# Shuijing725/CrowdNav_Prediction_AttnGraph

Measured on AMD Instinct MI355X. Metric: env-steps/sec (sim+policy fwd) at 20 humans, higher is better.
Workload: dtype f32 (big GEMMs as bf16x3 split-precision MFMA, fp32 accumulate); 1 GPU; BASELINE configs[1]: CrowdSimVarNum-v0, 20 humans, 4096 parallel envs per GPU, HH+HR attention on, policy forward + ORCA sim step + auto-reset per step; envs_per_gpu=4096, humans=20, parallelism=dp1 (envs sharded, no rollout collective), policy_init=orthogonal, torch.manual_seed(425), sampled_actions=True, side_stream_tail=inline, dephase_steps=240

## Files before the change

crowdnav_prediction_attngraph_amd/csrc/rn_fused.hip:

```cpp
#include "rn_fused.h"
#include "row_plan.h"

namespace {

typedef float f32x4 __attribute__((ext_vector_type(4)));
typedef __bf16 bf16x8 __attribute__((ext_vector_type(8)));

constexpr int TE = 16;
constexpr int S512 = 516, S384 = 388, S128 = 132;
constexpr int O_R0 = 0;
constexpr int O_R1 = O_R0 + TE * S512;
constexpr int O_R2 = O_R1 + TE * S512;
constexpr int O_R3 = O_R2 + TE * S384;
constexpr int O_R4 = O_R3 + TE * S384;
constexpr int O_R5 = O_R4 + TE * S128;
constexpr int LDS_FLOATS = O_R5 + TE * S128;

__device__ __forceinline__ f32x4 mfma32(bf16x8 a, bf16x8 b, f32x4 c) { return __builtin_amdgcn_mfma_f32_16x16x32_bf16(a, b, c, 0, 0, 0); }

enum { A_NONE = 0, A_RELU = 1, A_TANH = 2 };

__device__ __forceinline__ float fast_tanh(float x)
{
    const float e = __builtin_amdgcn_exp2f(x * 2.88539008177792681472f);
    return 1.0f - 2.0f / (1.0f + e);
}
__device__ __forceinline__ float fast_sigmoid(float x) { return 1.0f / (1.0f + __builtin_amdgcn_exp2f(x * -1.44269504088896340736f)); }

template <int K, int NFB, int ACT>
__device__ __forceinline__ void stage(const float *__restrict__ Wfrag_, int fb_first, int fb_step, const float *__restrict__ bias, const float *in, int in_stride,
                                      float *out, int out_stride, int out_off, int relu_from, int lane)
{
    const bf16x8 *__restrict__ Wfrag = reinterpret_cast<const bf16x8 *>(Wfrag_);
    const int i = lane & 15, g = lane >> 4;
    constexpr int KS = K / 32;
    bf16x8 bh, bl;
    auto split = [&](int ks, bf16x8 &h, bf16x8 &l) {
        const f32x4 x0 = *reinterpret_cast<const f32x4 *>(in + i * in_stride + 32 * ks + 8 * g);
        const f32x4 x1 = *reinterpret_cast<const f32x4 *>(in + i * in_stride + 32 * ks + 8 * g + 4);
#pragma unroll
        for (int u = 0; u < 4; ++u) {
            const __bf16 h0 = (__bf16)x0[u], h1 = (__bf16)x1[u];
            h[u] = h0; h[4 + u] = h1;
            l[u] = (__bf16)(x0[u] - (float)h0); l[4 + u] = (__bf16)(x1[u] - (float)h1);
        }
    };
    f32x4 acc[NFB];
#pragma unroll
    for (int j = 0; j < NFB; ++j) acc[j] = f32x4{0.f, 0.f, 0.f, 0.f};
    constexpr int PF = KS < 2 ? KS : 2;
    bf16x8 ah[PF][NFB], al[PF][NFB];
#pragma unroll
    for (int p = 0; p < PF - 1; ++p)
#pragma unroll
        for (int j = 0; j < NFB; ++j) {
            const size_t base = ((size_t)(fb_first + j * fb_step) * KS + (p < KS ? p : KS - 1)) * 128 + lane;
            ah[p][j] = Wfrag[base]; al[p][j] = Wfrag[base + 64];
        }
#pragma unroll
    for (int ks = 0; ks < KS; ++ks) {
        const int kp = ks + PF - 1 < KS ? ks + PF - 1 : KS - 1;
#pragma unroll
        for (int j = 0; j < NFB; ++j) {
            const size_t base = ((size_t)(fb_first + j * fb_step) * KS + kp) * 128 + lane;
            ah[(ks + PF - 1) % PF][j] = Wfrag[base]; al[(ks + PF - 1) % PF][j] = Wfrag[base + 64];
        }
        split(ks, bh, bl);
        __builtin_amdgcn_sched_barrier(0);
#pragma unroll
        for (int j = 0; j < NFB; ++j) {
            acc[j] = mfma32(al[ks % PF][j], bh, acc[j]);
            acc[j] = mfma32(ah[ks % PF][j], bl, acc[j]);
            acc[j] = mfma32(ah[ks % PF][j], bh, acc[j]);
        }
        __builtin_amdgcn_sched_barrier(0);
    }
#pragma unroll
    for (int j = 0; j < NFB; ++j) {
        const int f0 = (fb_first + j * fb_step) * 16 + 4 * g;
        f32x4 v = acc[j];
        if (bias) v += *reinterpret_cast<const f32x4 *>(bias + f0);
#pragma unroll
        for (int q = 0; q < 4; ++q) {
            if (ACT == A_RELU) { if (f0 + q >= relu_from) v[q] = fmaxf(v[q], 0.0f); }
            if (ACT == A_TANH) v[q] = fast_tanh(v[q]);
        }
        *reinterpret_cast<f32x4 *>(out + i * out_stride + out_off + f0) = v;
    }
}

__global__ __launch_bounds__(512, 4) void rn_fused_kernel(int E, int H, RnFusedArgs a)
{
    const CnStampScope stamp_scope(a.stamp);
    extern __shared__ __attribute__((aligned(16))) float smem[];
    __builtin_amdgcn_s_setprio(3);
    const int tid = threadIdx.x, lane = tid & 63, wave = __builtin_amdgcn_readfirstlane(tid >> 6);
    const int e0 = blockIdx.x * TE;
    float *R0 = smem + O_R0, *R1 = smem + O_R1, *R2 = smem + O_R2, *R3 = smem + O_R3, *R4 = smem + O_R4, *R5 = smem + O_R5;
    const int w4 = wave & 3, hi = wave >> 2;
    int r0q[2], r1q[2];
#pragma unroll
    for (int q = 0; q < 2; ++q) {
        const int e = e0 + 2 * wave + q < E ? e0 + 2 * wave + q : E - 1;
        r0q[q] = a.row_off[e]; r1q[q] = a.row_off[e + 1];
    }
    {
        const int n = tid & 255;
        float w[9];
#pragma unroll
        for (int d = 0; d < 9; ++d) w[d] = a.rl_w[n * 9 + d];
        const float bn = a.rl_b[n];
        for (int i = (tid >> 8) * (TE / 2); i < (tid >> 8) * (TE / 2) + TE / 2; ++i) {
            const int e = e0 + i < E ? e0 + i : E - 1;
            float acc = bn;
            acc += a.temporal[e * 2] * w[0];
            acc += a.temporal[e * 2 + 1] * w[1];
#pragma unroll
            for (int d = 0; d < 7; ++d) acc += a.robot_node[e * 7 + d] * w[2 + d];
            acc = fmaxf(acc, 0.0f);
            R0[i * S512 + n] = acc;
            if (a.tap_robot && e0 + i < E) a.tap_robot[(size_t)(e0 + i) * 256 + n] = acc;
        }
        for (int idx = tid; idx < TE * 128; idx += 512) {
            const int i = idx >> 7, c = idx & 127;
            const int e = e0 + i < E ? e0 + i : E - 1;
            R4[i * S128 + c] = a.hxs_in[(size_t)e * 128 + c];
        }
    }
#pragma unroll
    for (int q = 0; q < 2; ++q) { r0q[q] = held_uniform(r0q[q]); r1q[q] = held_uniform(r1q[q]); }
    __syncthreads();
    if (hi == 0) {
        stage<256, 3, A_RELU>(a.f_te, w4, 4, a.te_b, R0, S512, R1, S512, 0, 256, lane);
        stage<256, 2, A_RELU>(a.f_te, w4 + 12, 4, a.te_b, R0, S512, R1, S512, 0, 256, lane);
    } else {
        stage<128, 3, A_NONE>(a.f_whh, w4, 4, nullptr, R4, S128, R2, S384, 0, 0, lane);
        stage<128, 3, A_NONE>(a.f_whh, w4 + 12, 4, nullptr, R4, S128, R2, S384, 0, 0, lane);
    }
    __syncthreads();
    {
        constexpr int CH = 8;
        int ndq[2];
        float x[2][CH][4];
#pragma unroll
        for (int q = 0; q < 2; ++q) ndq[q] = r1q[q] - r0q[q];
#pragma unroll
        for (int q = 0; q < 2; ++q)
#pragma unroll
            for (int u = 0; u < CH; ++u) {
                const float *row = a.out_sp + (size_t)(r0q[q] + (u < ndq[q] ? u : ndq[q] - 1)) * 256;
                x[q][u][0] = row[lane]; x[q][u][1] = row[64 + lane]; x[q][u][2] = row[128 + lane]; x[q][u][3] = row[192 + lane];
            }
#pragma unroll
        for (int q = 0; q < 2; ++q) {
            const int i = 2 * wave + q;
            const int r0 = r0q[q], nd = ndq[q];
            const float *ue = R1 + i * S512;
            const float u0 = ue[lane], u1 = ue[64 + lane], u2 = ue[128 + lane], u3 = ue[192 + lane];
            float s = -INFINITY;
#pragma unroll
            for (int u = 0; u < CH; ++u) {
                const float tot = wv_sum(u0 * x[q][u][0] + u1 * x[q][u][1] + u2 * x[q][u][2] + u3 * x[q][u][3]);
                if (lane == u && u < nd) s = tot * ((float)H / 8.0f);
            }
            for (int j0 = CH; j0 < nd; j0 += CH) {
                float y[CH][4];
#pragma unroll
                for (int u = 0; u < CH; ++u) {
                    const float *row = a.out_sp + (size_t)(r0 + (j0 + u < nd ? j0 + u : nd - 1)) * 256;
                    y[u][0] = row[lane]; y[u][1] = row[64 + lane]; y[u][2] = row[128 + lane]; y[u][3] = row[192 + lane];
                }
#pragma unroll
                for (int u = 0; u < CH; ++u) {
                    const float tot = wv_sum(u0 * y[u][0] + u1 * y[u][1] + u2 * y[u][2] + u3 * y[u][3]);
                    if (lane == j0 + u && j0 + u < nd) s = tot * ((float)H / 8.0f);
                }
            }
            const float mx = wv_max(s);
            const float p = lane < nd ? expf(s - mx) : 0.0f;
            const float denom = wv_sum(p);
            const float at = p / denom;
            if (a.tap_attn && lane < H && e0 + i < E) a.tap_attn[(size_t)(e0 + i) * H + lane] = at;
            float o0 = 0.f, o1 = 0.f, o2 = 0.f, o3 = 0.f;
#pragma unroll
            for (int u = 0; u < CH; ++u) {
                const float aj = u < nd ? wv_readlane(at, u) : 0.0f;
                if (u < nd) { o0 += aj * x[q][u][0]; o1 += aj * x[q][u][1]; o2 += aj * x[q][u][2]; o3 += aj * x[q][u][3]; }
            }
            for (int j0 = CH; j0 < nd; j0 += CH) {
                float y[CH][4];
#pragma unroll
                for (int u = 0; u < CH; ++u) {
                    const float *row = a.out_sp + (size_t)(r0 + (j0 + u < nd ? j0 + u : nd - 1)) * 256;
                    y[u][0] = row[lane]; y[u][1] = row[64 + lane]; y[u][2] = row[128 + lane]; y[u][3] = row[192 + lane];
                }
#pragma unroll
                for (int u = 0; u < CH; ++u) {
                    const float aj = wv_readlane(at, j0 + u < nd ? j0 + u : 0);
                    if (j0 + u < nd) { o0 += aj * y[u][0]; o1 += aj * y[u][1]; o2 += aj * y[u][2]; o3 += aj * y[u][3]; }
                }
            }
            float *o = R0 + i * S512;
            o[lane] = o0; o[64 + lane] = o1; o[128 + lane] = o2; o[192 + lane] = o3;
            if (a.tap_hr && e0 + i < E) {
                float *t = a.tap_hr + (size_t)(e0 + i) * 256;
                t[lane] = o0; t[64 + lane] = o1; t[128 + lane] = o2; t[192 + lane] = o3;
            }
        }
    }
    __syncthreads();
    if (hi == 0) stage<256, 1, A_RELU>(a.f_edge, w4, 4, a.edge_b, R0, S512, R1, S512, 320, 0, lane);
    __syncthreads();
    stage<128, 3, A_NONE>(a.f_wih, wave, 8, a.bih, R1 + 256, S512, R3, S384, 0, 0, lane);
    __syncthreads();
    for (int idx = tid; idx < TE * 128; idx += 512) {
        const int i = idx >> 7, c = idx & 127;
        const int e = e0 + i < E ? e0 + i : E - 1;
        const float m = a.masks[e];
        const float *gie = R3 + i * S384, *ghe = R2 + i * S384;
        const float hr = m * ghe[c] + a.bhh[c], hz = m * ghe[128 + c] + a.bhh[128 + c], hn = m * ghe[256 + c] + a.bhh[256 + c];
        const float r = fast_sigmoid(gie[c] + hr);
        const float z = fast_sigmoid(gie[128 + c] + hz);
        const float n = fast_tanh(gie[256 + c] + r * hn);
        const float h = m * R4[i * S128 + c];
        const float hnew = (1.0f - z) * n + z * h;
        R5[i * S128 + c] = hnew;
        if (e0 + i < E) a.hxs_out[(size_t)(e0 + i) * 128 + c] = hnew;
    }
    __syncthreads();
    stage<128, 4, A_TANH>(a.f_ac0, wave, 8, a.ac0_b, R5, S128, R0, S512, 0, 0, lane);
    __syncthreads();
    {
        const float *fw = hi == 0 ? a.f_a2 : a.f_c2, *fb = hi == 0 ? a.a2_b : a.c2_b;
        const float *src = hi == 0 ? R0 : R0 + 256;
        stage<256, 2, A_TANH>(fw, w4, 4, fb, src, S512, R1, S512, hi * 256, 0, lane);
        stage<256, 2, A_TANH>(fw, w4 + 8, 4, fb, src, S512, R1, S512, hi * 256, 0, lane);
    }
    __syncthreads();
    for (int q = 0; q < 2; ++q) {
        const int i = 2 * wave + q;
        if (e0 + i >= E) break;
        const int e = e0 + i;
        const float *av = R1 + i * S512, *cv = av + 256;
        float sv = 0.f, s0 = 0.f, s1 = 0.f;
#pragma unroll
        for (int k = 0; k < 4; ++k) {
            const int d = lane + 64 * k;
            sv += cv[d] * a.cl_w[d];
            s0 += av[d] * a.fm_w[d];
            s1 += av[d] * a.fm_w[256 + d];
            if (a.tap_actor) a.tap_actor[(size_t)e * 256 + d] = av[d];
        }
        sv = wv_sum(sv); s0 = wv_sum(s0); s1 = wv_sum(s1);
        if (lane == 0) {
            a.value[e] = sv + a.cl_b[0];
            if (a.action) {
                const float mean0 = s0 + a.fm_b[0], mean1 = s1 + a.fm_b[1];
                const float ls0 = a.logstd[0], ls1 = a.logstd[1];
                const float sd0 = expf(ls0), sd1 = expf(ls1);
                const float a0 = a.eps ? mean0 + sd0 * a.eps[2 * e] : mean0;
                const float a1 = a.eps ? mean1 + sd1 * a.eps[2 * e + 1] : mean1;
                a.action[2 * e] = a0; a.action[2 * e + 1] = a1;
                const float HALF_LOG_2PI = 0.91893853320467274178f;
                const float d0 = a0 - mean0, d1 = a1 - mean1;
                a.logp[e] = (-(d0 * d0) / (2.0f * sd0 * sd0) - ls0 - HALF_LOG_2PI) + (-(d1 * d1) / (2.0f * sd1 * sd1) - ls1 - HALF_LOG_2PI);
            }
        }
    }
}

__global__ void rn_bake_kernel(int N, int K, const float *__restrict__ w, __bf16 *__restrict__ out)
{
    const size_t idx = (size_t)blockIdx.x * blockDim.x + threadIdx.x;
    if (idx >= (size_t)N * K) return;
    const int u = idx & 7, lane = (idx >> 3) & 63;
    const size_t rest = idx >> 9;
    const int KS = K / 32;
    const int ks = (int)(rest % KS), fb = (int)(rest / KS);
    const float x = w[(size_t)(fb * 16 + (lane & 15)) * K + 32 * ks + 8 * (lane >> 4) + u];
    const __bf16 hi = (__bf16)x;
    const size_t base = (((size_t)fb * KS + ks) * 2) * 512 + lane * 8 + u;
    out[base] = hi;
    out[base + 512] = (__bf16)(x - (float)hi);
}

}

int rn_fused_bake(int N, int K, const float *w, float *out, hipStream_t st)
{
    CN_REQUIRE(N % 16 == 0 && K % 32 == 0, "rn_fused_bake: N must be a multiple of 16, K of 32");
    const size_t n = (size_t)N * K;
    hipLaunchKernelGGL(rn_bake_kernel, dim3((unsigned)((n + 255) / 256)), dim3(256), 0, st, N, K, w, reinterpret_cast<__bf16 *>(out));
    CN_CHECK_LAUNCH();
    return CN_OK;
}

int rn_fused_forward(int E, int H, const RnFusedArgs &args, hipStream_t st)
{
    constexpr size_t lds = (size_t)LDS_FLOATS * sizeof(float);
    static thread_local int attr_dev = -1;
    int dev = 0;
    CN_HIP(hipGetDevice(&dev));
    if (dev != attr_dev) {
        CN_HIP(hipFuncSetAttribute(reinterpret_cast<const void *>(&rn_fused_kernel), hipFuncAttributeMaxDynamicSharedMemorySize, (int)lds));
        attr_dev = dev;
    }
    RnFusedArgs a = args;
    a.stamp = cn_stamp_slot(CN_K_RN_FUSED);
    hipLaunchKernelGGL(rn_fused_kernel, dim3((E + TE - 1) / TE), dim3(512), lds, st, E, H, a);
    CN_CHECK_LAUNCH();
    return CN_OK;
}
```

Before: 15.65 million env-steps/s.

## Preload biases, head weights and per-env scalars into LDS; rebalance GEMM waves

All biases, head weights, masks, eps and small scalars are loaded once at kernel start into a new LDS region, with loads issued up front and held in registers, replacing scattered global reads later in the kernel. Robot-node inputs are loaded per wave and broadcast with readlane. The first stage now splits work 5/3 across waves between the te and whh GEMMs, and the a2/c2 stage uses one call with four fragment blocks. Tap writes are compiled out through a template flag. The cost is more LDS per block and more register pressure up front.

```diff
diff --git a/crowdnav_prediction_attngraph_amd/csrc/rn_fused.hip b/crowdnav_prediction_attngraph_amd/csrc/rn_fused.hip
--- a/crowdnav_prediction_attngraph_amd/csrc/rn_fused.hip
+++ b/crowdnav_prediction_attngraph_amd/csrc/rn_fused.hip
@@ -14,7 +14,15 @@
 constexpr int O_R3 = O_R2 + TE * S384;
 constexpr int O_R4 = O_R3 + TE * S384;
 constexpr int O_R5 = O_R4 + TE * S128;
-constexpr int LDS_FLOATS = O_R5 + TE * S128;
+constexpr int O_T = O_R5 + TE * S128;
+constexpr int T_TEB = 0, T_EDGEB = T_TEB + 320, T_BIH = T_EDGEB + 64, T_BHH = T_BIH + 384, T_AC0B = T_BHH + 384, T_A2B = T_AC0B + 512;
+constexpr int T_C2B = T_A2B + 256, T_CLW = T_C2B + 256, T_FMW = T_CLW + 256;
+constexpr int T_VEC4 = (T_FMW + 512) / 4;
+constexpr int T_SM = T_FMW + 512;
+constexpr int SM_MASK = 0, SM_EPS = 16, SM_CLB = 48, SM_FMB = 49, SM_LS = 51, SM_WORDS = 53;
+constexpr int T_FLOATS = T_SM + 64;
+constexpr int LDS_FLOATS = O_T + T_FLOATS;
+static_assert(LDS_FLOATS * sizeof(float) <= 160 * 1024, "rn_fused: LDS");
 
 __device__ __forceinline__ f32x4 mfma32(bf16x8 a, bf16x8 b, f32x4 c) { return __builtin_amdgcn_mfma_f32_16x16x32_bf16(a, b, c, 0, 0, 0); }
 
@@ -27,8 +35,8 @@
 }
 __device__ __forceinline__ float fast_sigmoid(float x) { return 1.0f / (1.0f + __builtin_amdgcn_exp2f(x * -1.44269504088896340736f)); }
 
-template <int K, int NFB, int ACT>
-__device__ __forceinline__ void stage(const float *__restrict__ Wfrag_, int fb_first, int fb_step, const float *__restrict__ bias, const float *in, int in_stride,
+template <int K, int NFB, int ACT, bool BIAS>
+__device__ __forceinline__ void stage(const float *__restrict__ Wfrag_, int fb_first, int fb_step, const float *bias, const float *in, int in_stride,
                                       float *out, int out_stride, int out_off, int relu_from, int lane)
 {
     const bf16x8 *__restrict__ Wfrag = reinterpret_cast<const bf16x8 *>(Wfrag_);
@@ -79,7 +87,7 @@
     for (int j = 0; j < NFB; ++j) {
         const int f0 = (fb_first + j * fb_step) * 16 + 4 * g;
         f32x4 v = acc[j];
-        if (bias) v += *reinterpret_cast<const f32x4 *>(bias + f0);
+        if (BIAS) v += *reinterpret_cast<const f32x4 *>(bias + f0);
 #pragma unroll
         for (int q = 0; q < 4; ++q) {
             if (ACT == A_RELU) { if (f0 + q >= relu_from) v[q] = fmaxf(v[q], 0.0f); }
@@ -89,6 +97,7 @@
     }
 }
 
+template <bool TAPS>
 __global__ __launch_bounds__(512, 4) void rn_fused_kernel(int E, int H, RnFusedArgs a)
 {
     const CnStampScope stamp_scope(a.stamp);
@@ -96,7 +105,7 @@
     __builtin_amdgcn_s_setprio(3);
     const int tid = threadIdx.x, lane = tid & 63, wave = __builtin_amdgcn_readfirstlane(tid >> 6);
     const int e0 = blockIdx.x * TE;
-    float *R0 = smem + O_R0, *R1 = smem + O_R1, *R2 = smem + O_R2, *R3 = smem + O_R3, *R4 = smem + O_R4, *R5 = smem + O_R5;
+    float *R0 = smem + O_R0, *R1 = smem + O_R1, *R2 = smem + O_R2, *R3 = smem + O_R3, *R4 = smem + O_R4, *R5 = smem + O_R5, *T = smem + O_T;
     const int w4 = wave & 3, hi = wave >> 2;
     int r0q[2], r1q[2];
 #pragma unroll
@@ -104,38 +113,97 @@
         const int e = e0 + 2 * wave + q < E ? e0 + 2 * wave + q : E - 1;
         r0q[q] = a.row_off[e]; r1q[q] = a.row_off[e + 1];
     }
-    {
-        const int n = tid & 255;
-        float w[9];
-#pragma unroll
-        for (int d = 0; d < 9; ++d) w[d] = a.rl_w[n * 9 + d];
-        const float bn = a.rl_b[n];
-        for (int i = (tid >> 8) * (TE / 2); i < (tid >> 8) * (TE / 2) + TE / 2; ++i) {
-            const int e = e0 + i < E ? e0 + i : E - 1;
+    const int n = tid & 255;
+    float w[9];
+#pragma unroll
+    for (int d = 0; d < 9; ++d) w[d] = a.rl_w[n * 9 + d];
+    float bn = a.rl_b[n];
+    float obs_t, obs_r;
+    {
+        const int lt = lane < 16 ? lane : 15, lr = lane < 56 ? lane : 55;
+        const int it = e0 + 8 * hi + (lt >> 1), ir = e0 + 8 * hi + lr / 7;
+        obs_t = a.temporal[(size_t)(it < E ? it : E - 1) * 2 + (lt & 1)];
+        obs_r = a.robot_node[(size_t)(ir < E ? ir : E - 1) * 7 + lr % 7];
+    }
+    float hx[4];
+#pragma unroll
+    for (int k = 0; k < 4; ++k) {
+        const int i = (tid >> 7) + 4 * k;
+        hx[k] = a.hxs_in[(size_t)(e0 + i < E ? e0 + i : E - 1) * 128 + (tid & 127)];
+    }
+    f32x4 tv[2];
+    {
+        const float *const p_teb = a.te_b, *const p_edgeb = a.edge_b, *const p_bih = a.bih, *const p_bhh = a.bhh, *const p_ac0b = a.ac0_b;
+        const float *const p_a2b = a.a2_b, *const p_c2b = a.c2_b, *const p_clw = a.cl_w, *const p_fmw = a.fm_w;
+#pragma unroll
+        for (int r = 0; r < 2; ++r) {
+            const int j = 512 * r + tid < T_VEC4 ? 512 * r + tid : T_VEC4 - 1, f = 4 * j;
+            const float *src = p_teb; int first = T_TEB;
+            src = f >= T_EDGEB ? p_edgeb : src; first = f >= T_EDGEB ? T_EDGEB : first;
+            src = f >= T_BIH ? p_bih : src; first = f >= T_BIH ? T_BIH : first;
+            src = f >= T_BHH ? p_bhh : src; first = f >= T_BHH ? T_BHH : first;
+            src = f >= T_AC0B ? p_ac0b : src; first = f >= T_AC0B ? T_AC0B : first;
+            src = f >= T_A2B ? p_a2b : src; first = f >= T_A2B ? T_A2B : first;
+            src = f >= T_C2B ? p_c2b : src; first = f >= T_C2B ? T_C2B : first;
+            src = f >= T_CLW ? p_clw : src; first = f >= T_CLW ? T_CLW : first;
+            src = f >= T_FMW ? p_fmw : src; first = f >= T_FMW ? T_FMW : first;
+            tv[r] = *reinterpret_cast<const f32x4 *>(src + (f - first));
+        }
+    }
+    float smw;
+    {
+        const float *const p_masks = a.masks, *const p_eps = a.eps, *const p_clb = a.cl_b, *const p_fmb = a.fm_b, *const p_ls = a.logstd;
+        const bool has_eps = p_eps != nullptr;
+        const int sl = lane < SM_WORDS ? lane : SM_WORDS - 1;
+        const int i = sl < SM_EPS ? sl : (sl - SM_EPS) >> 1;
+        const int e = e0 + i < E ? e0 + i : E - 1;
+        const bool is_eps = sl >= SM_EPS && has_eps;
+        const float *src = is_eps ? p_eps : p_masks; int off = is_eps ? 2 * e + (sl & 1) : e;
+        src = sl >= SM_CLB ? p_clb : src; off = sl >= SM_CLB ? 0 : off;
+        src = sl >= SM_FMB ? p_fmb : src; off = sl >= SM_FMB ? sl - SM_FMB : off;
+        src = sl >= SM_LS ? p_ls : src; off = sl >= SM_LS ? sl - SM_LS : off;
+        smw = src[off];
+    }
+#pragma unroll
+    for (int d = 0; d < 9; ++d) w[d] = held(w[d]);
+    bn = held(bn); obs_t = held(obs_t); obs_r = held(obs_r); smw = held(smw);
+#pragma unroll
+    for (int k = 0; k < 4; ++k) hx[k] = held(hx[k]);
+#pragma unroll
+    for (int r = 0; r < 2; ++r) tv[r] = held(tv[r]);
+#pragma unroll
+    for (int q = 0; q < 2; ++q) { r0q[q] = held_uniform(r0q[q]); r1q[q] = held_uniform(r1q[q]); }
+    *reinterpret_cast<f32x4 *>(T + 4 * tid) = tv[0];
+    if (512 + tid < T_VEC4) *reinterpret_cast<f32x4 *>(T + 4 * (512 + tid)) = tv[1];
+    if (wave == 0) T[T_SM + lane] = smw;
+#pragma unroll
+    for (int k = 0; k < 4; ++k) R4[((tid >> 7) + 4 * k) * S128 + (tid & 127)] = hx[k];
+    {
+        float rs[TE / 2];
+#pragma unroll
+        for (int ii = 0; ii < TE / 2; ++ii) {
             float acc = bn;
-            acc += a.temporal[e * 2] * w[0];
-            acc += a.temporal[e * 2 + 1] * w[1];
-#pragma unroll
-            for (int d = 0; d < 7; ++d) acc += a.robot_node[e * 7 + d] * w[2 + d];
-            acc = fmaxf(acc, 0.0f);
-            R0[i * S512 + n] = acc;
-            if (a.tap_robot && e0 + i < E) a.tap_robot[(size_t)(e0 + i) * 256 + n] = acc;
-        }
-        for (int idx = tid; idx < TE * 128; idx += 512) {
-            const int i = idx >> 7, c = idx & 127;
-            const int e = e0 + i < E ? e0 + i : E - 1;
-            R4[i * S128 + c] = a.hxs_in[(size_t)e * 128 + c];
-        }
-    }
-#pragma unroll
-    for (int q = 0; q < 2; ++q) { r0q[q] = held_uniform(r0q[q]); r1q[q] = held_uniform(r1q[q]); }
-    __syncthreads();
-    if (hi == 0) {
-        stage<256, 3, A_RELU>(a.f_te, w4, 4, a.te_b, R0, S512, R1, S512, 0, 256, lane);
-        stage<256, 2, A_RELU>(a.f_te, w4 + 12, 4, a.te_b, R0, S512, R1, S512, 0, 256, lane);
+            acc += wv_readlane(obs_t, 2 * ii) * w[0];
+            acc += wv_readlane(obs_t, 2 * ii + 1) * w[1];
+#pragma unroll
+            for (int d = 0; d < 7; ++d) acc += wv_readlane(obs_r, 7 * ii + d) * w[2 + d];
+            rs[ii] = fmaxf(acc, 0.0f);
+            R0[(8 * hi + ii) * S512 + n] = rs[ii];
+        }
+        if (TAPS) {
+#pragma unroll
+            for (int ii = 0; ii < TE / 2; ++ii) {
+                const int i = 8 * hi + ii;
+                if (e0 + i < E) a.tap_robot[(size_t)(e0 + i) * 256 + n] = rs[ii];
+            }
+        }
+    }
+    __syncthreads();
+    if (wave < 5) {
+        stage<256, 4, A_RELU, true>(a.f_te, wave, 5, T + T_TEB, R0, S512, R1, S512, 0, 256, lane);
     } else {
-        stage<128, 3, A_NONE>(a.f_whh, w4, 4, nullptr, R4, S128, R2, S384, 0, 0, lane);
-        stage<128, 3, A_NONE>(a.f_whh, w4 + 12, 4, nullptr, R4, S128, R2, S384, 0, 0, lane);
+        stage<128, 4, A_NONE, false>(a.f_whh, wave - 5, 3, nullptr, R4, S128, R2, S384, 0, 0, lane);
+        stage<128, 4, A_NONE, false>(a.f_whh, wave - 5 + 12, 3, nullptr, R4, S128, R2, S384, 0, 0, lane);
     }
     __syncthreads();
     {
@@ -180,7 +248,6 @@
             const float p = lane < nd ? expf(s - mx) : 0.0f;
             const float denom = wv_sum(p);
             const float at = p / denom;
-            if (a.tap_attn && lane < H && e0 + i < E) a.tap_attn[(size_t)(e0 + i) * H + lane] = at;
             float o0 = 0.f, o1 = 0.f, o2 = 0.f, o3 = 0.f;
 #pragma unroll
             for (int u = 0; u < CH; ++u) {
@@ -202,69 +269,72 @@
             }
             float *o = R0 + i * S512;
             o[lane] = o0; o[64 + lane] = o1; o[128 + lane] = o2; o[192 + lane] = o3;
-            if (a.tap_hr && e0 + i < E) {
+            if (TAPS && e0 + i < E) {
+                if (lane < H) a.tap_attn[(size_t)(e0 + i) * H + lane] = at;
                 float *t = a.tap_hr + (size_t)(e0 + i) * 256;
                 t[lane] = o0; t[64 + lane] = o1; t[128 + lane] = o2; t[192 + lane] = o3;
             }
         }
     }
     __syncthreads();
-    if (hi == 0) stage<256, 1, A_RELU>(a.f_edge, w4, 4, a.edge_b, R0, S512, R1, S512, 320, 0, lane);
-    __syncthreads();
-    stage<128, 3, A_NONE>(a.f_wih, wave, 8, a.bih, R1 + 256, S512, R3, S384, 0, 0, lane);
-    __syncthreads();
-    for (int idx = tid; idx < TE * 128; idx += 512) {
-        const int i = idx >> 7, c = idx & 127;
-        const int e = e0 + i < E ? e0 + i : E - 1;
-        const float m = a.masks[e];
-        const float *gie = R3 + i * S384, *ghe = R2 + i * S384;
-        const float hr = m * ghe[c] + a.bhh[c], hz = m * ghe[128 + c] + a.bhh[128 + c], hn = m * ghe[256 + c] + a.bhh[256 + c];
+    if (hi == 0) stage<256, 1, A_RELU, true>(a.f_edge, w4, 4, T + T_EDGEB, R0, S512, R1, S512, 320, 0, lane);
+    __syncthreads();
+    stage<128, 3, A_NONE, true>(a.f_wih, wave, 8, T + T_BIH, R1 + 256, S512, R3, S384, 0, 0, lane);
+    __syncthreads();
+#pragma unroll
+    for (int k = 0; k < 4; ++k) {
+        const int i = (tid >> 7) + 4 * k, c = tid & 127;
+        const float m = T[T_SM + SM_MASK + i];
+        const float *gie = R3 + i * S384, *ghe = R2 + i * S384, *bhh = T + T_BHH;
+        const float hr = m * ghe[c] + bhh[c], hz = m * ghe[128 + c] + bhh[128 + c], hn = m * ghe[256 + c] + bhh[256 + c];
         const float r = fast_sigmoid(gie[c] + hr);
         const float z = fast_sigmoid(gie[128 + c] + hz);
-        const float n = fast_tanh(gie[256 + c] + r * hn);
+        const float nn = fast_tanh(gie[256 + c] + r * hn);
         const float h = m * R4[i * S128 + c];
-        const float hnew = (1.0f - z) * n + z * h;
+        const float hnew = (1.0f - z) * nn + z * h;
         R5[i * S128 + c] = hnew;
         if (e0 + i < E) a.hxs_out[(size_t)(e0 + i) * 128 + c] = hnew;
     }
     __syncthreads();
-    stage<128, 4, A_TANH>(a.f_ac0, wave, 8, a.ac0_b, R5, S128, R0, S512, 0, 0, lane);
-    __syncthreads();
-    {
-        const float *fw = hi == 0 ? a.f_a2 : a.f_c2, *fb = hi == 0 ? a.a2_b : a.c2_b;
+    stage<128, 4, A_TANH, true>(a.f_ac0, wave, 8, T + T_AC0B, R5, S128, R0, S512, 0, 0, lane);
+    __syncthreads();
+    {
+        const float *fw = hi == 0 ? a.f_a2 : a.f_c2, *fb = hi == 0 ? T + T_A2B : T + T_C2B;
         const float *src = hi == 0 ? R0 : R0 + 256;
-        stage<256, 2, A_TANH>(fw, w4, 4, fb, src, S512, R1, S512, hi * 256, 0, lane);
-        stage<256, 2, A_TANH>(fw, w4 + 8, 4, fb, src, S512, R1, S512, hi * 256, 0, lane);
+        stage<256, 4, A_TANH, true>(fw, w4, 4, fb, src, S512, R1, S512, hi * 256, 0, lane);
     }
     __syncthreads();
     for (int q = 0; q < 2; ++q) {
         const int i = 2 * wave + q;
         if (e0 + i >= E) break;
         const int e = e0 + i;
-        const float *av = R1 + i * S512, *cv = av + 256;
+        const float *av = R1 + i * S512, *cv = av + 256, *cl_w = T + T_CLW, *fm_w = T + T_FMW, *sm = T + T_SM;
         float sv = 0.f, s0 = 0.f, s1 = 0.f;
 #pragma unroll
         for (int k = 0; k < 4; ++k) {
             const int d = lane + 64 * k;
-            sv += cv[d] * a.cl_w[d];
-            s0 += av[d] * a.fm_w[d];
-            s1 += av[d] * a.fm_w[256 + d];
-            if (a.tap_actor) a.tap_actor[(size_t)e * 256 + d] = av[d];
+            sv += cv[d] * cl_w[d];
+            s0 += av[d] * fm_w[d];
+            s1 += av[d] * fm_w[256 + d];
         }
         sv = wv_sum(sv); s0 = wv_sum(s0); s1 = wv_sum(s1);
         if (lane == 0) {
-            a.value[e] = sv + a.cl_b[0];
+            a.value[e] = sv + sm[SM_CLB];
             if (a.action) {
-                const float mean0 = s0 + a.fm_b[0], mean1 = s1 + a.fm_b[1];
-                const float ls0 = a.logstd[0], ls1 = a.logstd[1];
+                const float mean0 = s0 + sm[SM_FMB], mean1 = s1 + sm[SM_FMB + 1];
+                const float ls0 = sm[SM_LS], ls1 = sm[SM_LS + 1];
                 const float sd0 = expf(ls0), sd1 = expf(ls1);
-                const float a0 = a.eps ? mean0 + sd0 * a.eps[2 * e] : mean0;
-                const float a1 = a.eps ? mean1 + sd1 * a.eps[2 * e + 1] : mean1;
+                const float a0 = a.eps ? mean0 + sd0 * sm[SM_EPS + 2 * i] : mean0;
+                const float a1 = a.eps ? mean1 + sd1 * sm[SM_EPS + 2 * i + 1] : mean1;
                 a.action[2 * e] = a0; a.action[2 * e + 1] = a1;
                 const float HALF_LOG_2PI = 0.91893853320467274178f;
                 const float d0 = a0 - mean0, d1 = a1 - mean1;
                 a.logp[e] = (-(d0 * d0) / (2.0f * sd0 * sd0) - ls0 - HALF_LOG_2PI) + (-(d1 * d1) / (2.0f * sd1 * sd1) - ls1 - HALF_LOG_2PI);
             }
+        }
+        if (TAPS) {
+#pragma unroll
+            for (int k = 0; k < 4; ++k) a.tap_actor[(size_t)e * 256 + lane + 64 * k] = av[lane + 64 * k];
         }
     }
 }
@@ -295,19 +365,30 @@
     return CN_OK;
 }
 
-int rn_fused_forward(int E, int H, const RnFusedArgs &args, hipStream_t st)
+template <bool TAPS>
+static int rn_fused_launch(int E, int H, const RnFusedArgs &a, hipStream_t st)
 {
     constexpr size_t lds = (size_t)LDS_FLOATS * sizeof(float);
     static thread_local int attr_dev = -1;
     int dev = 0;
     CN_HIP(hipGetDevice(&dev));
     if (dev != attr_dev) {
-        CN_HIP(hipFuncSetAttribute(reinterpret_cast<const void *>(&rn_fused_kernel), hipFuncAttributeMaxDynamicSharedMemorySize, (int)lds));
+        CN_HIP(hipFuncSetAttribute(reinterpret_cast<const void *>(&rn_fused_kernel<TAPS>), hipFuncAttributeMaxDynamicSharedMemorySize, (int)lds));
         attr_dev = dev;
     }
+    hipLaunchKernelGGL(rn_fused_kernel<TAPS>, dim3((E + TE - 1) / TE), dim3(512), lds, st, E, H, a);
+    CN_CHECK_LAUNCH();
+    return CN_OK;
+}
+
+int rn_fused_forward(int E, int H, const RnFusedArgs &args, hipStream_t st)
+{
+    CN_REQUIRE(E >= 1, "rn_fused_forward: E must be positive");
+    const bool taps = args.tap_robot || args.tap_attn || args.tap_hr || args.tap_actor;
+    CN_REQUIRE(!taps || (args.tap_robot && args.tap_attn && args.tap_hr && args.tap_actor), "rn_fused_forward: the four taps come together");
+    for (const float *p : {args.te_b, args.edge_b, args.bih, args.bhh, args.ac0_b, args.a2_b, args.c2_b, args.cl_w, args.fm_w})
+        CN_REQUIRE(p && ((uintptr_t)p & 15) == 0, "rn_fused_forward: biases and head weights must be 16-byte aligned");
     RnFusedArgs a = args;
     a.stamp = cn_stamp_slot(CN_K_RN_FUSED);
-    hipLaunchKernelGGL(rn_fused_kernel, dim3((E + TE - 1) / TE), dim3(512), lds, st, E, H, a);
-    CN_CHECK_LAUNCH();
-    return CN_OK;
-}
+    return taps ? rn_fused_launch<true>(E, H, a, st) : rn_fused_launch<false>(E, H, a, st);
+}
```

Measured after the change: 15.83 million env-steps/s (median of 6 runs). 1.01x the previous value.
